# backtato/ai-video-detector

Hardware: AMD Instinct MI355X
Metric: sampled frames/sec analysed (1080p30 60 s clip, 2 fps sampling) (higher is better)
Workload: dtype u8 pixels; f32/f64 Farneback (cv2's own types); 1 GPU; BASELINE.json configs[1]: 1080p30 60 s clip, 2 fps sampling, one clip per GPU per step; frames_per_clip=120, height=1080, width=1920, clips_in_flight_per_gpu=3, fb_mode=fast+rerun, fb_wide160=2, parallelism=single GPU, rccl_ranks_seen=1

## Files before the change

ai-video-detector_amd/csrc/avd_capi.hip:

```cpp
#include <algorithm>
#include <cstdlib>
#include <atomic>
#include <cstring>
#include <new>
#include <thread>
#include "avd_internal.h"

namespace {

constexpr int kFbChunk = 128;
constexpr int kFbChunkMax = 512;

struct TableBlob {
    std::vector<uint8_t> bytes;
    template <typename T>
    size_t push(const std::vector<T>& v)
    {
        size_t off = (bytes.size() + 15) / 16 * 16;
        bytes.resize(off + v.size() * sizeof(T));
        std::memcpy(bytes.data() + off, v.data(), v.size() * sizeof(T));
        return off;
    }
};

// ... 741 lines not shown
        avd_ctx* c;
        ~Uncount() { if (c->counted_in_flight) { c->counted_in_flight = 0; g_calls_in_flight.fetch_sub(1, std::memory_order_relaxed); } }
    } uncount{ctx};
    HIP_TRY(ctx, hipSetDevice(ctx->device));
    if (ctx->tail.active) {
        const hipError_t e = ctx->tail_registered ? wait_helping(ctx, ctx->tail_ev) : hipStreamSynchronize(ctx->stream);
        tail_unregister(ctx);
        if (e != hipSuccess) { ctx->tail.active = 0; ctx->pending_out = nullptr; ctx->pending_n = 0; ctx->err = hipGetErrorString(e); return AVD_ERR_DEVICE; }
        if (ctx->tail.active) ctx->tail_rc = tail_settle(ctx);
    }
    if (ctx->tail_rc) {
        const int rc = ctx->tail_rc;
        ctx->tail_rc = 0; ctx->pending_out = nullptr; ctx->pending_n = 0;
        return rc;
    }
    HIP_TRY(ctx, wait_helping(ctx, nullptr));
    if (ctx->pending_out) {
        const avd_frame_record* const got = ctx->ws.h_rec + ctx->pending_off;
        std::memcpy(ctx->pending_out, got, sizeof(avd_frame_record) * ctx->pending_n);
        ctx->last_rerun = 0;
        for (int i = 0; i < ctx->pending_n; i++) ctx->last_rerun += got[i].reserved != 0;
        ctx->pending_out = nullptr; ctx->pending_n = 0;
    }
    if (ctx->profiling && ctx->kmark_used > 1 && ctx->kmark_id[ctx->kmark_used - 1] == AVD_K_COUNT) {
        for (float& v : ctx->kernel_ms) v = 0.f;
        for (int i = 0; i + 1 < ctx->kmark_used; i++) {
            float ms = 0.f;
            if (ctx->kmark_id[i] < AVD_K_COUNT && hipEventElapsedTime(&ms, ctx->kmark_at[i], ctx->kmark_at[i + 1]) == hipSuccess)
                ctx->kernel_ms[ctx->kmark_id[i]] += ms;
        }
        ctx->kmark_incomplete = ctx->kmark_overflow;
    }
    kmark_reset(ctx);
    if (ctx->profiling && ctx->stage_marks == 5) {
        for (int i = 0; i < 4; i++) {
            float ms = 0.f;
            if (hipEventElapsedTime(&ms, ctx->stage_ev[i], ctx->stage_ev[i + 1]) == hipSuccess) ctx->stage_ms[i] = ms;
        }
        float sum[2] = {0.f, 0.f}; int cnt[2] = {0, 0};
        for (int i = 0; i + 1 < ctx->kern_ev_used; i += 2) {
            float ms = 0.f;
            if (hipEventElapsedTime(&ms, ctx->kern_ev[i], ctx->kern_ev[i + 1]) == hipSuccess) { sum[(i >> 1) & 1] += ms; cnt[(i >> 1) & 1]++; }
        }
        for (int k = 0; k < 2; k++) ctx->stage_ms[4 + k] = cnt[k] ? sum[k] / cnt[k] : 0.f;
        ctx->stage_marks = 0;
    }
    return AVD_OK;
}

static int impl_timer_start(avd_ctx* ctx)
{
    if (!ctx) return AVD_ERR_ARG;
    HIP_TRY(ctx, hipEventRecord(ctx->ev0, ctx->stream));
    return AVD_OK;
}

static int impl_timer_stop(avd_ctx* ctx, float* elapsed_ms)
{
    if (!ctx || !elapsed_ms) return AVD_ERR_ARG;
    HIP_TRY(ctx, hipEventRecord(ctx->ev1, ctx->stream));
    HIP_TRY(ctx, hipEventSynchronize(ctx->ev1));
    HIP_TRY(ctx, hipEventElapsedTime(elapsed_ms, ctx->ev0, ctx->ev1));
    return AVD_OK;
}

static int impl_set_profiling(avd_ctx* ctx, int enable)
{
    if (!ctx) return AVD_ERR_ARG;
    ctx->profiling = enable != 0;
    return AVD_OK;
}

static int impl_stage_ms(avd_ctx* ctx, int stage, float* ms)
{
    if (!ctx || !ms || stage < 0 || stage > 5) return AVD_ERR_ARG;
    *ms = ctx->stage_ms[stage];
    return AVD_OK;
}

static int impl_kernel_ms(avd_ctx* ctx, int id, float* ms)
{
    if (!ctx || !ms || id < 0 || id >= AVD_K_COUNT) return AVD_ERR_ARG;
    if (ctx->kmark_incomplete) { ctx->err = "avd_kernel_ms: the profiled call had more kernel regions than the library records (96): split it"; return AVD_ERR_ARG; }
    *ms = ctx->kernel_ms[id];
    return AVD_OK;
}

static int64_t impl_debug_fetch(avd_ctx* ctx, const char* name, void* out, size_t out_bytes)
{
    if (!ctx || !name || !out) return AVD_ERR_ARG;
    Workspace& ws = ctx->ws;
    const int n = ctx->last_n;
    const void* src = nullptr;
    size_t bytes = 0;
    auto level = [&](const char* prefix) -> int {
        const size_t L = std::strlen(prefix);
        if (std::strncmp(name, prefix, L) == 0 && name[L] >= '0' && name[L] < '0' + AVD_FB_LEVELS && name[L + 1] == 0)
            return name[L] - '0';
        return -1;
    };
    int k;
    {
        const IngestRecord& in = ctx->ingest;
        const char* const no_launch = "no ingest kernel was launched on this context";
        const char* const no_call = "no ingest call has run on this context";
        const struct { const char* name; const void* p; size_t bytes; bool recorded; const char* missing; const char* type; } host_state[] = {
            {"ingest_plan", &in.plan, sizeof in.plan, in.launched != 0, no_launch, nullptr},
            {"ingest_rotate", &in.rotate, sizeof in.rotate, in.launched != 0, no_launch, "int32[1]"},
            {"ingest_range", &in.range, sizeof in.range, in.launched != 0, no_launch, "int32[1]"},
            {"ingest_format", &in.format, sizeof in.format, in.launched != 0, no_launch, "int32[1]"},
            {"ingest_list", in.list, sizeof in.list, in.launched != 0, no_launch, "int32[2]"},
            {"stage_copies", &in.stage_copies, sizeof in.stage_copies, in.stage_copies >= 0, no_call, "int64[1]"},
            {"stage_bytes", &in.stage_bytes, sizeof in.stage_bytes, in.stage_bytes >= 0, no_call, "int64[1]"},
        };
        for (const auto& e : host_state) {
            if (std::strcmp(name, e.name) != 0) continue;
            if (!e.recorded) { ctx->err = std::string(e.name) + " not recorded yet: " + e.missing; return AVD_ERR_ARG; }
            if (e.type && out_bytes < e.bytes) { ctx->err = std::string(e.name) + " is " + e.type; return AVD_ERR_ARG; }
            bytes = std::min(e.bytes, out_bytes);
            std::memcpy(out, e.p, bytes);
            return (int64_t)bytes;
        }
    }
    if (std::strcmp(name, "cnn_plan") == 0) {
        if (!ctx->cnn_plan_valid) { ctx->err = "cnn_plan not recorded yet: no CNN forward has run on this context"; return AVD_ERR_ARG; }
        bytes = std::min(sizeof(ctx->cnn_plan), out_bytes);
        std::memcpy(out, ctx->cnn_plan, bytes);
        return (int64_t)bytes;
    }
    if (std::strcmp(name, "cnn_tap") == 0) {
        HIP_TRY(ctx, hipSetDevice(ctx->device));
        return cnn_tap_fetch(ctx, out, out_bytes);
    }
    if (std::strncmp(name, "audio_", 6) == 0) {
        const bool plan = std::strcmp(name + 6, "plan") == 0, xw = std::strcmp(name + 6, "xw") == 0, mag = std::strcmp(name + 6, "mag") == 0;
        if (!plan && !xw && !mag) { ctx->err = "unknown debug buffer"; return AVD_ERR_ARG; }
        if (!ctx->audio_plan_valid) { ctx->err = "audio_plan / audio_xw / audio_mag not recorded yet: no avd_audio_features call has run on this context"; return AVD_ERR_ARG; }
        if (plan) {
            if (out_bytes < sizeof(ctx->audio_plan)) { ctx->err = "audio_plan is int32[4]"; return AVD_ERR_ARG; }
            std::memcpy(out, ctx->audio_plan, sizeof(ctx->audio_plan));
            return (int64_t)sizeof(ctx->audio_plan);
        }
        const size_t nwin = (size_t)ctx->audio_plan[0], win = (size_t)ctx->audio_plan[1];
        if (!ws.d_audio_buf) { ctx->err = "buffer not allocated yet"; return AVD_ERR_ARG; }
        src = xw ? ws.d_audio_buf.p : ws.d_audio_buf.p + nwin * win;
        bytes = (xw ? nwin * win : nwin * (win / 2 + 1)) * sizeof(double);
    }
    else if (std::strcmp(name, "area") == 0) { src = ws.d_area; bytes = (size_t)n * 1024; }
    else if (std::strcmp(name, "small") == 0) { src = ws.d_small; bytes = (size_t)n * AVD_NPIX; }
    else if ((k = level("pyr")) >= 0 && k == 0 && ctx->fb_fold_blur) { ctx->err = "pyr0 does not exist while fb_fold_blur is on (the polynomial expansion forms the 320-px blur itself)"; return AVD_ERR_ARG; }
    else if ((k = level("pyr")) >= 0) { src = ws.d_pyr[k]; bytes = (size_t)std::min(n, ws.fb_cap + 1) * (AVD_NPIX >> (2 * k)) * 4; }
    else if ((k = level("poly")) >= 0) { src = ws.d_poly[k]; bytes = (size_t)std::min(n, ws.fb_cap + 1) * 5 * (AVD_NPIX >> (2 * k)) * 4; }
    else if ((k = level("flow")) >= 0) { src = ws.fb_holds.flow[k] ? ws.fb_holds.flow[k] : ws.d_flow[k]; bytes = (size_t)std::min(std::max(n - 1, 0), ws.fb_cap) * 2 * (AVD_NPIX >> (2 * k)) * 4; }
    else if (std::strcmp(name, "vs0") == 0) { src = ws.d_vs0; bytes = fb_two_scratch_size((size_t)ws.fb_cap).vs0 * sizeof(double); }
    else { ctx->err = "unknown debug buffer"; return AVD_ERR_ARG; }
    if (!src) { ctx->err = "buffer not allocated yet"; return AVD_ERR_ARG; }
    bytes = std::min(bytes, out_bytes);
    HIP_TRY(ctx, hipSetDevice(ctx->device));
    HIP_TRY(ctx, hipStreamSynchronize(ctx->stream));
    HIP_TRY(ctx, hipMemcpy(out, src, bytes, hipMemcpyDeviceToHost));
    return (int64_t)bytes;
}

static int impl_wait_stream(avd_ctx* ctx, void* producer)
{
    if (!ctx) return AVD_ERR_ARG;
    HIP_TRY(ctx, hipSetDevice(ctx->device));
    HIP_TRY(ctx, hipEventRecord(ctx->ev_in, (hipStream_t)producer));
    HIP_TRY(ctx, hipStreamWaitEvent(ctx->stream, ctx->ev_in, 0));
    return AVD_OK;
}

static int impl_release_workspace(avd_ctx* ctx)
{
    if (!ctx) return AVD_ERR_ARG;
    HIP_TRY(ctx, hipSetDevice(ctx->device));
    if (int e = impl_synchronize(ctx)) return e;
    ctx->ws = Workspace{};
    ctx->rec_n = 0;
    return AVD_OK;
}

static int impl_set_option(avd_ctx* ctx, const char* name, int value)
{
    if (!ctx || !name) return AVD_ERR_ARG;
    const Option* o = find_option(ctx, name, true);
    if (!o) return AVD_ERR_ARG;
    if (!o->norm(value)) { ctx->err = o->refused; return AVD_ERR_ARG; }
    if (o->act) o->act(ctx, value);
    else ctx->*o->field = value;
    return AVD_OK;
}

static int impl_get_option(avd_ctx* ctx, const char* name, int* value)
{
    if (!ctx || !name || !value) return AVD_ERR_ARG;
    const Option* o = find_option(ctx, name, false);
    if (!o) return AVD_ERR_ARG;
    *value = o->read ? o->read(ctx) : ctx->*o->field;
    return AVD_OK;
}

template <typename F>
static int time_reps(avd_ctx* ctx, int reps, F&& launch, float* out_ms)
{
    HIP_TRY(ctx, hipEventRecord(ctx->ev0, ctx->stream));
    for (int r = 0; r < reps; r++)
        if (int e = launch()) return e;
    HIP_TRY(ctx, hipEventRecord(ctx->ev1, ctx->stream));
    HIP_TRY(ctx, hipEventSynchronize(ctx->ev1));
    float ms = 0.f;
    HIP_TRY(ctx, hipEventElapsedTime(&ms, ctx->ev0, ctx->ev1));
    *out_ms = ms / reps;
    return 0;
}

static int impl_cnn_set_weights(avd_ctx* ctx, const uint16_t* w, size_t n_w, const float* b, size_t n_b)
{
    if (!ctx || !w || !b) return AVD_ERR_ARG;
    size_t want_w = 0, want_b = 0;
    cnn_param_counts(&want_w, &want_b);
    if (n_w != want_w || n_b != want_b) { ctx->err = "avd_cnn_set_weights: parameter counts differ from avd_cnn_param_counts"; return AVD_ERR_ARG; }
    HIP_TRY(ctx, hipSetDevice(ctx->device));
    return cnn_set_weights(ctx, w, b);
}

static int impl_cnn_forward(avd_ctx* ctx, const uint8_t* bgr, int mem, int n, int h, int w, int64_t row_stride, int64_t frame_stride,
                            float* logits, int reps, float* forward_ms)
{
    if (!ctx) return AVD_ERR_ARG;
    if ((!bgr || !logits) && n > 0) { ctx->err = "null pointer"; return AVD_ERR_ARG; }
    if (n < 0 || h < 2 || w < 2 || row_stride < (int64_t)w * 3) { ctx->err = "bad frame geometry"; return AVD_ERR_ARG; }
    if (n == 0) return AVD_OK;
    HIP_TRY(ctx, hipSetDevice(ctx->device));
    Workspace& ws = ctx->ws;
    if (!ctx->weights.d_cnn_w) { ctx->err = "avd_cnn_set_weights has not been called"; return AVD_ERR_ARG; }
    const int kChunk = ctx->cnn_chunk;
    if (ctx->cnn_tap && (n > kChunk || reps > 0)) { ctx->err = "avd_cnn_forward: with option cnn_tap set, one pass (n <= cnn_chunk) and no timing repetitions"; return AVD_ERR_ARG; }
    if (int e = cnn_reserve(ctx, std::min(n, kChunk))) return e;
    const uint8_t* d_bgr = nullptr;
    if (int e = stage_input(ctx, bgr, mem, plane_span(frame_stride, n, row_stride, h, (size_t)w * 3), &d_bgr)) return e;
    float total_ms = 0.f;
    for (int f0 = 0; f0 < n; f0 += kChunk) {
        const int m = std::min(kChunk, n - f0);
        const uint8_t* src = d_bgr + (size_t)frame_stride * f0;
        auto forward = [&] { return launch_cnn_forward(ctx, src, m, h, w, row_stride, frame_stride); };
        if (int e = forward()) return e;
        if (reps > 0 && forward_ms) {
            float ms = 0.f;
            if (int e = time_reps(ctx, reps, forward, &ms)) return e;
            total_ms += ms;
        }
        HIP_TRY(ctx, hipMemcpyAsync(logits + (size_t)f0 * 1000, ws.d_cnn_logits, sizeof(float) * (size_t)m * 1000, hipMemcpyDeviceToHost, ctx->stream));
    }
    if (reps > 0 && forward_ms) *forward_ms = total_ms;
    HIP_TRY(ctx, hipStreamSynchronize(ctx->stream));
    return AVD_OK;
}

static int impl_vit_set_weights(avd_ctx* ctx, const uint16_t* w_bf16, const float* bias)
{
    if (!ctx || !w_bf16) return AVD_ERR_ARG;
    HIP_TRY(ctx, hipSetDevice(ctx->device));
    Weights& wt = ctx->weights;
    if (int e = wt.d_vit_w.reserve(ctx, (size_t)768 * 768)) return e;
    if (int e = wt.d_vit_bias.reserve(ctx, (size_t)768)) return e;
    std::vector<uint16_t> blocked((size_t)768 * 768);
    gemm_block_operand(w_bf16, blocked.data(), 768, 768);
    HIP_TRY(ctx, hipMemcpyAsync(wt.d_vit_w, blocked.data(), sizeof(uint16_t) * 768 * 768, hipMemcpyHostToDevice, ctx->stream));
    if (bias) HIP_TRY(ctx, hipMemcpyAsync(wt.d_vit_bias, bias, sizeof(float) * 768, hipMemcpyHostToDevice, ctx->stream));
    wt.vit_has_bias = bias != nullptr;
    HIP_TRY(ctx, hipStreamSynchronize(ctx->stream));
    return AVD_OK;
}

static int impl_vit_patch_embed(avd_ctx* ctx, const uint8_t* bgr, int mem, int n, int h, int w, int64_t row_stride,
                                int64_t frame_stride, void* tokens, int tokens_mem, int tokens_bf16, int reps, float* gemm_ms)
{
    if (!ctx) return AVD_ERR_ARG;
    if ((!bgr || !tokens) && n > 0) { ctx->err = "null pointer"; return AVD_ERR_ARG; }
    if (n < 0 || h < 2 || w < 2 || row_stride < (int64_t)w * 3) { ctx->err = "bad frame geometry"; return AVD_ERR_ARG; }
    if (tokens_mem != AVD_MEM_HOST && tokens_mem != AVD_MEM_DEVICE) { ctx->err = "tokens_mem must be AVD_MEM_HOST or AVD_MEM_DEVICE"; return AVD_ERR_ARG; }
    if (n == 0) return AVD_OK;
    HIP_TRY(ctx, hipSetDevice(ctx->device));
    Workspace& ws = ctx->ws;
    const Weights& wt = ctx->weights;
    if (!wt.d_vit_w) { ctx->err = "avd_vit_set_weights has not been called"; return AVD_ERR_ARG; }
    const size_t m = (size_t)n * 196;
    const size_t m_pad = (m + kGemmRowPad - 1) / kGemmRowPad * kGemmRowPad;
    if (ws.d_vit_patches.cap < m_pad * 768) {
        if (int e = ws.d_vit_patches.reserve(ctx, m_pad * 768)) return e;
        auto zero_fill = [&]() -> int { HIP_TRY(ctx, hipMemsetAsync(ws.d_vit_patches, 0, m_pad * 768 * sizeof(uint16_t), ctx->stream)); return 0; };
        if (int e = zero_fill()) { ws.d_vit_patches.reset(); return e; }
    }
    void* d_tok = tokens;
    const size_t esz = tokens_bf16 ? sizeof(uint16_t) : sizeof(float);
    if (tokens_mem == AVD_MEM_HOST) {
        if (int e = ws.d_vit_tokens.reserve(ctx, m * 768)) return e;
        d_tok = ws.d_vit_tokens;
    }
    const uint8_t* d_bgr = nullptr;
    if (int e = stage_input(ctx, bgr, mem, plane_span(frame_stride, n, row_stride, h, (size_t)w * 3), &d_bgr)) return e;
    const float* d_bias = wt.vit_has_bias ? wt.d_vit_bias : nullptr;
    if (int e = launch_vit_patch_embed(ctx, d_bgr, n, h, w, row_stride, frame_stride, wt.d_vit_w, d_bias, d_tok, tokens_bf16, ws.d_vit_patches)) return e;
    if (reps > 0 && gemm_ms) {
        auto gemm = [&] { return launch_gemm_bf16_nt(ctx, ws.d_vit_patches, wt.d_vit_w, d_bias, d_tok, tokens_bf16, (int)m, 768, 768); };
// ... 345 lines not shown
```

ai-video-detector_amd/csrc/avd_farneback.hip:

```cpp
#include "avd_internal.h"
#include "avd_fb_device.h"

#pragma clang fp contract(off)

namespace {

constexpr int S = AVD_SMALL;

template <int K>
struct PyrGeo {
    static constexpr int WL = S >> K;
    static constexpr int NC = K == 0 ? S : 2 * WL;
    static constexpr int OFF = K == 0 ? 0 : (1 << K) / 2 - 1;
    static constexpr int TR = K >= 2 ? 4 : 8;
    static constexpr int TILES = WL / TR;
    static constexpr int KS = K == 3 ? 19 : (K == 2 ? 9 : 3), HALF = KS / 2;
    static constexpr int SROWS = K == 0 ? TR + 2 * HALF : ((TR - 1) << K) + 2 + 2 * HALF;
    static constexpr int PADX = 12, PS = S + 2 * PADX;
    static constexpr int SRC_BYTES = SROWS * PS, LDS_BYTES = SRC_BYTES + SROWS * NC * 4;
};
constexpr int cmax(int a, int b) { return a > b ? a : b; }
constexpr int cgcd(int a, int b) { return b == 0 ? a : cgcd(b, a % b); }

template <int PR>
struct PyrWalk {
    static constexpr int PER = PR / cgcd(256, PR), SG = 256 / cgcd(256, PR);
    __device__ static __forceinline__ void first(int tid, int& r, int& c)
    {
        r = 0; c = tid;
#pragma unroll
        for (int q = 1; q * PR < 256; q++)
            if (tid >= q * PR) { r = q; c = tid - q * PR; }
    }
    __device__ static __forceinline__ void next(int& r, int& c)
    {
        r += 256 / PR; c += 256 % PR;
        if (c >= PR) { c -= PR; r++; }
    }
};
constexpr int kPyrLds = cmax(cmax(PyrGeo<3>::LDS_BYTES, PyrGeo<2>::LDS_BYTES), cmax(PyrGeo<1>::LDS_BYTES, PyrGeo<0>::LDS_BYTES));

template <int K>
__device__ __forceinline__ void pyramid_body(char* lds, int blk, const uint8_t* __restrict__ small, const FbConsts* __restrict__ C,
                                             float* __restrict__ I, int n = 0, int* __restrict__ pairdiff = nullptr)
{
    using G = PyrGeo<K>;
    constexpr int WL = G::WL, NC = G::NC, OFF = G::OFF, TR = G::TR, KS = G::KS, HALF = G::HALF, SROWS = G::SROWS;
    constexpr int PADX = G::PADX, PS = G::PS;
    uint8_t (*src)[PS] = reinterpret_cast<uint8_t (*)[PS]>(lds);
    float (*rowf)[NC] = reinterpret_cast<float (*)[NC]>(lds + G::SRC_BYTES);
    const int tiles = WL / TR;
    const int f = blk / tiles, t = blk - f * tiles;
    const int tid = threadIdx.x;
    const int dy0 = t * TR;
    const int y_first = (K == 0 ? dy0 : (dy0 << K) + OFF) - HALF;
    const uint8_t* img = small + (int64_t)f * AVD_NPIX;
    const bool cmp = K == 1 && pairdiff != nullptr && f + 1 < n;
    int differs = 0;
    for (int it = tid; it < SROWS * (S / 4); it += 256) {
        const int r = it / (S / 4), c4 = it - r * (S / 4);
        const int y = reflect101(y_first + r, S);
        const unsigned v = reinterpret_cast<const unsigned*>(img + y * S)[c4];
        reinterpret_cast<unsigned*>(src[r] + PADX)[c4] = v;
        if (K == 1 && cmp) differs |= v != reinterpret_cast<const unsigned*>(img + AVD_NPIX + y * S)[c4];
    }
    for (int it = tid; it < SROWS * 2 * HALF; it += 256) {
        const int r = it / (2 * HALF), i = it - r * (2 * HALF);
        const uint8_t* g = img + reflect101(y_first + r, S) * S;
        if (i < HALF) src[r][PADX - 1 - i] = g[1 + i];
        else src[r][PADX + S + (i - HALF)] = g[S - 2 - (i - HALF)];
    }
    if (K == 1 && cmp) {
        const int any = __syncthreads_or(differs);
        if (tid == 0) pairdiff[f * tiles + t] = any;
    } else
        __syncthreads();
    float kw[KS];
#pragma unroll
    for (int q = 0; q < KS; q++) kw[q] = C->gk[K][q];
    if (KS == 3) {
        static_assert(KS != 3 || NC == S, "the 3-tap scales filter whole rows");
        using W = PyrWalk<S / 4>;
        typedef float f4 __attribute__((ext_vector_type(4)));
        const unsigned* wp0[W::PER]; f4* dst0[W::PER]; int r0[W::PER];
        {
            int r, c4;
            W::first(tid, r, c4);
#pragma unroll
            for (int i = 0; i < W::PER; i++) {
                r0[i] = r;
                wp0[i] = reinterpret_cast<const unsigned*>(src[r] + PADX + 4 * c4);
                dst0[i] = reinterpret_cast<f4*>(&rowf[r][4 * c4]);
                W::next(r, c4);
            }
        }
        for (int sb = 0; sb < SROWS; sb += W::SG) {
#pragma unroll
            for (int i = 0; i < W::PER; i++) {
                if (256 * i >= SROWS * (S / 4) || r0[i] + sb >= SROWS) continue;
                const unsigned* wp = wp0[i] + sb * (PS / 4);
                const unsigned pw = wp[-1], cwd = wp[0], nw = wp[1];
                const float b[6] = {(float)(pw >> 24), (float)(cwd & 0xFFu), (float)((cwd >> 8) & 0xFFu), (float)((cwd >> 16) & 0xFFu),
                                    (float)(cwd >> 24), (float)(nw & 0xFFu)};
                f4 o;
#pragma unroll
                for (int e = 0; e < 4; e++) o[e] = __builtin_fmaf(b[e + 1], kw[1], (b[e] + b[e + 2]) * kw[0]);
                dst0[i][sb * (NC / 4)] = o;
            }
        }
    } else {
        using W = PyrWalk<NC>;
        constexpr int NW = (KS + 3) / 4;
        const unsigned* wp0[W::PER]; float* dst0[W::PER]; int r0[W::PER], sh0[W::PER];
        {
            int r, j;
            W::first(tid, r, j);
#pragma unroll
            for (int i = 0; i < W::PER; i++) {
                const int x = K == 0 ? j : ((j >> 1) << K) + OFF + (j & 1);
                const int base = PADX + x - HALF;
                r0[i] = r; sh0[i] = base & 3;
                wp0[i] = reinterpret_cast<const unsigned*>(src[r] + (base & ~3));
                dst0[i] = &rowf[r][j];
                W::next(r, j);
            }
        }
        for (int sb = 0; sb < SROWS; sb += W::SG) {
#pragma unroll
            for (int i = 0; i < W::PER; i++) {
                if (256 * i >= SROWS * NC || r0[i] + sb >= SROWS) continue;
                const unsigned* wp = wp0[i] + sb * (PS / 4);
                unsigned d[NW + 1];
#pragma unroll
                for (int q = 0; q <= NW; q++) d[q] = wp[q];
                float v = 0.f;
#pragma unroll
                for (int q = 0; q < NW; q++) {
                    const unsigned wv = __builtin_amdgcn_alignbyte(d[q + 1], d[q], sh0[i]);
#pragma unroll
                    for (int e = 0; e < 4; e++)
                        if (q * 4 + e < KS) v = __builtin_fmaf((float)((wv >> (8 * e)) & 0xFFu), kw[q * 4 + e], v);
                }
                dst0[i][sb * NC] = v;
            }
        }
    }
    __syncthreads();
    auto colf = [&](const float* c) {
        float sacc = __builtin_fmaf(c[0], kw[HALF], 0.f);
#pragma unroll
        for (int k = 1; k <= HALF; k++) sacc = __builtin_fmaf(c[k * NC] + c[-k * NC], kw[HALF + k], sacc);
        return sacc;
    };
    {
        using W = PyrWalk<WL>;
        float* out = I + ((int64_t)f * WL + dy0) * WL;
        int dyl, dx;
        W::first(tid, dyl, dx);
#pragma unroll
        for (int i = 0; i < W::PER; i++) {
            if (256 * i < TR * WL) {
                for (int y = dyl; y < TR; y += W::SG) {
                    float o;
                    if (K == 0) {
                        o = colf(&rowf[y + HALF][dx]);
                    } else {
                        const float* c = &rowf[(y << K) + HALF][2 * dx];
                        const float p00 = colf(c), p01 = colf(c + 1);
                        const float p10 = colf(c + NC), p11 = colf(c + NC + 1);
                        o = ((p00 + p01) + (p10 + p11)) * 0.25f;
                    }
                    out[y * WL + dx] = o;
                }
            }
            W::next(dyl, dx);
        }
    }
}

__global__ __launch_bounds__(256) void k_pyramid_all(const uint8_t* __restrict__ small, int n, const FbConsts* __restrict__ C,
                                                    float* __restrict__ I0, float* __restrict__ I1, float* __restrict__ I2,
                                                    float* __restrict__ I3, int* __restrict__ flags, int* __restrict__ pairdiff)
{
    static_assert(PyrGeo<1>::TILES == kPairDiffTiles, "avd_fbfast.hip reads one word per 160-px tile");
    __shared__ __align__(16) char lds[kPyrLds];
    if (flags && (int)(blockIdx.x * 256 + threadIdx.x) < n - 1) flags[blockIdx.x * 256 + threadIdx.x] = 0;
    const int n3 = n * PyrGeo<3>::TILES, n2 = n * PyrGeo<2>::TILES, n1 = n * PyrGeo<1>::TILES;
    int b = blockIdx.x;
    if (b < n3) { pyramid_body<3>(lds, b, small, C, I3); return; }
    b -= n3;
    if (b < n2) { pyramid_body<2>(lds, b, small, C, I2); return; }
    b -= n2;
    if (b < n1) { pyramid_body<1>(lds, b, small, C, I1, n, pairdiff); return; }
    if (I0) pyramid_body<0>(lds, b - n1, small, C, I0);
}

struct PolyPtrs { const float* I[AVD_FB_LEVELS]; float* R[AVD_FB_LEVELS]; const uint8_t* small; };

constexpr int kPolyRows = 16;
constexpr int kPolyQuads = 4 * (S / 4 + 10);
static_assert(AVD_FB_LEVELS == 4, "three walking scales and the one-row form of the coarsest");
__host__ __device__ constexpr int poly_wgs(int k) { return k < AVD_FB_LEVELS - 1 ? (S >> k) / kPolyRows : S >> (2 * k); }

typedef float pf4 __attribute__((ext_vector_type(4)));
typedef float pf2 __attribute__((ext_vector_type(2)));

__device__ __forceinline__ void polyexp_put(pf4* __restrict__ rowq, int x, int w, float t0, float t1, float t2)
{
    const pf4 t = {t0, t1, t1, t2};
    rowq[x + 5] = t;
    if (x == 0)
        for (int q = 0; q < 5; q++) rowq[q] = t;
    if (x == w - 1)
        for (int q = 0; q < 5; q++) rowq[w + 5 + q] = t;
}

__device__ __forceinline__ void polyexp_hpass(const pf4* __restrict__ rq, const float (&g)[6], const float (&xg)[6], const double (&gd)[6],
                                              const double (&xxgd)[6], double ig11, double ig03, double ig33, double ig55, float* __restrict__ o)
{
    const pf4 c = rq[0];
    double b1 = (double)(c.x * g[0]), b2 = 0, b3 = (double)(c.y * g[0]), b4 = 0, b5 = (double)(c.w * g[0]), b6 = 0;
#pragma unroll
    for (int q = 1; q <= 5; q++) {
        const pf4 p = rq[q], m = rq[-q];
        const pf2 s01 = p.xy + m.xy, d01 = p.xy - m.xy, s12 = p.zw + m.zw;
        const pf2 dx = d01 * pf2{xg[q], xg[q]};
        const pf2 sg = s12 * pf2{g[q], g[q]};
        const double tg = (double)s01.x;
        b1 = __builtin_fma(tg, gd[q], b1);
        b4 = __builtin_fma(tg, xxgd[q], b4);
        b2 += (double)dx.x;
        b3 += (double)sg.x;
        b6 += (double)dx.y;
        b5 += (double)sg.y;
    }
    o[0] = (float)(b3 * ig11);
    o[1] = (float)(b2 * ig11);
    o[2] = (float)(b1 * ig03 + b5 * ig33);
    o[3] = (float)(b1 * ig03 + b4 * ig33);
    o[4] = (float)(b6 * ig55);
}

template <int K, bool FOLD>
__device__ __forceinline__ void polyexp_rows(const float* __restrict__ img, const uint8_t* __restrict__ small, float* __restrict__ out, int y0,
                                             const FbConsts* __restrict__ C, pf4 (*rowb)[kPolyQuads], float (*outb)[S * 5])
{
    static_assert(!FOLD || K == 0, "only the 320-px scale forms its own blur");
    constexpr int w = S >> K, h = w, R = 1 << K, STEPS = kPolyRows / R;
    static_assert(R * (w + 10) <= kPolyQuads && h % kPolyRows == 0 && kPolyRows % R == 0, "a step's R rows fit one LDS buffer; whole bands");
    const int tid = threadIdx.x;
    const int sr = K == 0 ? 0 : tid / w, x = tid - sr * w;
    const int yb = y0 + sr;
    const int xs = x - 1 < 0 ? 0 : (x - 1 > w - 4 ? w - 4 : x - 1);
    const int shl = ((x == 0 ? 1 : x - 1) - xs) * 8, shc = (x - xs) * 8, shr = ((x == w - 1 ? w - 2 : x + 1) - xs) * 8;
    const float kx0 = C->gk[0][0], kx1 = C->gk[0][1], kx2 = C->gk[0][2];
    struct __attribute__((packed, aligned(1))) U4 { unsigned v; };
    auto hb = [&](int srow) __attribute__((always_inline)) {
        const int sr = srow < 0 ? -srow : (srow > h - 1 ? 2 * (h - 1) - srow : srow);
        const unsigned wd = reinterpret_cast<const U4*>(small + sr * w + xs)->v;
        const float l = (float)((wd >> shl) & 0xFFu), c = (float)((wd >> shc) & 0xFFu), r = (float)((wd >> shr) & 0xFFu);
        return __builtin_fmaf(c, kx1, (l + r) * kx0);
    };
    float hm = 0.f, h0 = 0.f, hp = 0.f;
    int rcur = -1000;
    auto blurred = [&](int r) __attribute__((always_inline)) {
        if (r != rcur) {
            if (r == rcur + 1) { hm = h0; h0 = hp; hp = hb(r + 1); }
            else { hm = hb(r - 1); h0 = hb(r); hp = hb(r + 1); }
            rcur = r;
        }
        return __builtin_fmaf(hp + hm, kx2, __builtin_fmaf(h0, kx1, 0.f));
    };
    auto pixel = [&](int r) __attribute__((always_inline)) { return FOLD ? blurred(r) : img[r * w + x]; };
    typedef float f4 __attribute__((ext_vector_type(4)));
    typedef float f2 __attribute__((ext_vector_type(2)));
    float g[6], xg[6], xxg[6];
    double gd[6], xxgd[6];
#pragma unroll
    for (int q = 0; q <= 5; q++) { g[q] = C->g[5 + q]; xg[q] = C->xg[5 + q]; xxg[q] = C->xxg[5 + q]; gd[q] = C->gd[q]; xxgd[q] = C->xxgd[q]; }
    const double ig11 = C->ig11, ig03 = C->ig03, ig33 = C->ig33, ig55 = C->ig55;
    float win[11 + kPolyRows - R];
#pragma unroll
    for (int q = 0; q < 10; q++) win[q] = pixel(min(max(yb - 5 + q, 0), h - 1));
    pf4* rowq[2] = {rowb[0] + sr * (w + 10), rowb[1] + sr * (w + 10)};
#pragma unroll
    for (int i = 0; i < STEPS; i++) {
        const int par = i & 1, o = R * i;
#pragma unroll
        for (int j = o + 11 - R; j <= o + 10; j++)
            if (j >= 10) win[j] = pixel(min(yb - 5 + j, h - 1));
        {
            f2 t02 = f2{win[o + 5] * g[0], 0.f};
            float t1 = 0.f;
#pragma unroll
            for (int q = 1; q <= 5; q++) {
                const float a = win[o + 5 - q], bb = win[o + 5 + q];
                const float p = a + bb;
                t02 = t02 + f2{g[q], xxg[q]} * f2{p, p};
                t1 = t1 + xg[q] * (bb - a);
            }
            polyexp_put(rowq[par], x, w, t02.x, t1, t02.y);
        }
        __syncthreads();
        if (i > 0) {
            f4* dst = reinterpret_cast<f4*>(out + (int64_t)(y0 + o - R) * w * 5);
            const f4* srcv = reinterpret_cast<const f4*>(outb[par ^ 1]);
            __builtin_nontemporal_store(srcv[tid], dst + tid);
            if (tid < S * 5 / 4 - 320) __builtin_nontemporal_store(srcv[tid + 320], dst + tid + 320);
        }
        polyexp_hpass(rowq[par] + x + 5, g, xg, gd, xxgd, ig11, ig03, ig33, ig55, outb[par] + tid * 5);
    }
    __syncthreads();
    {
        f4* dst = reinterpret_cast<f4*>(out + (int64_t)(y0 + kPolyRows - R) * w * 5);
        const f4* srcv = reinterpret_cast<const f4*>(outb[(STEPS - 1) & 1]);
        __builtin_nontemporal_store(srcv[tid], dst + tid);
        if (tid < S * 5 / 4 - 320) __builtin_nontemporal_store(srcv[tid + 320], dst + tid + 320);
    }
}

__global__ __launch_bounds__(320) void k_polyexp_all(PolyPtrs P, int n, const FbConsts* __restrict__ C)
{
    __shared__ pf4 rowb[2][kPolyQuads];
    __shared__ __align__(16) float outbb[2][S * 5];
    pf4* row = rowb[0];
    static_assert(8 * (S / 8 + 10) <= 2 * kPolyQuads, "the eight sub-rows of the coarsest scale fit");
    float* outb = outbb[0];
    int b = (int)blockIdx.x, k = 0, wgs = 0;
    for (; k < AVD_FB_LEVELS; k++) {
        wgs = n * poly_wgs(k);
        const int cnt = ((wgs + 7) >> 3) << 3;
// ... 336 lines not shown
```

Measured before the change: 145,100 frames/s.

## Reuse horizontally filtered halo rows across two vertical steps in pyramid levels 2-3

```diff
diff --git a/ai-video-detector_amd/csrc/avd_capi.hip b/ai-video-detector_amd/csrc/avd_capi.hip
--- a/ai-video-detector_amd/csrc/avd_capi.hip
+++ b/ai-video-detector_amd/csrc/avd_capi.hip
@@ -917,6 +917,7 @@
     else if ((k = level("pyr")) >= 0) { src = ws.d_pyr[k]; bytes = (size_t)std::min(n, ws.fb_cap + 1) * (AVD_NPIX >> (2 * k)) * 4; }
     else if ((k = level("poly")) >= 0) { src = ws.d_poly[k]; bytes = (size_t)std::min(n, ws.fb_cap + 1) * 5 * (AVD_NPIX >> (2 * k)) * 4; }
     else if ((k = level("flow")) >= 0) { src = ws.fb_holds.flow[k] ? ws.fb_holds.flow[k] : ws.d_flow[k]; bytes = (size_t)std::min(std::max(n - 1, 0), ws.fb_cap) * 2 * (AVD_NPIX >> (2 * k)) * 4; }
+    else if (std::strcmp(name, "pairdiff") == 0) { src = ws.d_pairdiff; bytes = (size_t)std::min(std::max(n - 1, 0), ws.fb_cap) * kPairDiffTiles * sizeof(int); }
     else if (std::strcmp(name, "vs0") == 0) { src = ws.d_vs0; bytes = fb_two_scratch_size((size_t)ws.fb_cap).vs0 * sizeof(double); }
     else { ctx->err = "unknown debug buffer"; return AVD_ERR_ARG; }
     if (!src) { ctx->err = "buffer not allocated yet"; return AVD_ERR_ARG; }
diff --git a/ai-video-detector_amd/csrc/avd_farneback.hip b/ai-video-detector_amd/csrc/avd_farneback.hip
--- a/ai-video-detector_amd/csrc/avd_farneback.hip
+++ b/ai-video-detector_amd/csrc/avd_farneback.hip
@@ -13,11 +13,17 @@
     static constexpr int NC = K == 0 ? S : 2 * WL;
     static constexpr int OFF = K == 0 ? 0 : (1 << K) / 2 - 1;
     static constexpr int TR = K >= 2 ? 4 : 8;
-    static constexpr int TILES = WL / TR;
+    static constexpr int STEPS = K >= 2 ? 2 : 1, BAND = STEPS * TR;
+    static constexpr int TILES = WL / BAND;
     static constexpr int KS = K == 3 ? 19 : (K == 2 ? 9 : 3), HALF = KS / 2;
     static constexpr int SROWS = K == 0 ? TR + 2 * HALF : ((TR - 1) << K) + 2 + 2 * HALF;
+    static constexpr int NEW = K == 0 ? TR : TR << K, KEEP = SROWS - NEW;
     static constexpr int PADX = 12, PS = S + 2 * PADX;
     static constexpr int SRC_BYTES = SROWS * PS, LDS_BYTES = SRC_BYTES + SROWS * NC * 4;
+    static constexpr int FILTERED_PCT = TILES * (SROWS + (STEPS - 1) * NEW) * 100 / S;
+    static_assert(WL % BAND == 0 && (K == 0 || FILTERED_PCT <= 120), "whole bands; a source row is filtered at most 1.2 times per frame");
+    static_assert(STEPS == 1 || (KEEP * NC <= 4 * 256 && SRC_BYTES % 16 == 0 && (NEW * NC) % 4 == 0 && (KEEP * NC) % 4 == 0),
+                  "the rows a step takes over move as one 16-byte piece per lane");
 };
 constexpr int cmax(int a, int b) { return a > b ? a : b; }
 constexpr int cgcd(int a, int b) { return b == 0 ? a : cgcd(b, a % b); }
@@ -40,49 +46,71 @@
 };
 constexpr int kPyrLds = cmax(cmax(PyrGeo<3>::LDS_BYTES, PyrGeo<2>::LDS_BYTES), cmax(PyrGeo<1>::LDS_BYTES, PyrGeo<0>::LDS_BYTES));
 
+typedef float pyr_f4 __attribute__((ext_vector_type(4)));
+typedef float pyr_f2 __attribute__((ext_vector_type(2)));
+
 template <int K>
-__device__ __forceinline__ void pyramid_body(char* lds, int blk, const uint8_t* __restrict__ small, const FbConsts* __restrict__ C,
-                                             float* __restrict__ I, int n = 0, int* __restrict__ pairdiff = nullptr)
+__device__ __forceinline__ void pyramid_step(char* lds, const uint8_t* __restrict__ img, const float (&kw)[PyrGeo<K>::KS], float* __restrict__ out,
+                                             int y_first, int rb, pyr_f4& kept, bool more, int* __restrict__ diffword)
 {
     using G = PyrGeo<K>;
     constexpr int WL = G::WL, NC = G::NC, OFF = G::OFF, TR = G::TR, KS = G::KS, HALF = G::HALF, SROWS = G::SROWS;
     constexpr int PADX = G::PADX, PS = G::PS;
     uint8_t (*src)[PS] = reinterpret_cast<uint8_t (*)[PS]>(lds);
     float (*rowf)[NC] = reinterpret_cast<float (*)[NC]>(lds + G::SRC_BYTES);
-    const int tiles = WL / TR;
-    const int f = blk / tiles, t = blk - f * tiles;
     const int tid = threadIdx.x;
-    const int dy0 = t * TR;
-    const int y_first = (K == 0 ? dy0 : (dy0 << K) + OFF) - HALF;
-    const uint8_t* img = small + (int64_t)f * AVD_NPIX;
-    const bool cmp = K == 1 && pairdiff != nullptr && f + 1 < n;
+    const bool cmp = K == 1 && diffword != nullptr;
+    static_assert(K != 1 || G::STEPS == 1, "the pair-identity word is formed by a tile that loads all its source rows in one step");
+    static_assert(HALF + 1 < S, "a source row is reflected at most once");
+    auto row_at = [&](int r) -> unsigned { const int y = y_first + r; return (unsigned)(y < 0 ? -y : (y >= S ? 2 * S - 2 - y : y)) * S; };
+    constexpr int NLD = (SROWS * (S / 4) + 255) / 256, NBD = (SROWS * 2 * HALF + 255) / 256;
+    const int nld = (SROWS - rb) * (S / 4), nbd = (SROWS - rb) * 2 * HALF;
+    constexpr int NBATCH = 8;
     int differs = 0;
-    for (int it = tid; it < SROWS * (S / 4); it += 256) {
-        const int r = it / (S / 4), c4 = it - r * (S / 4);
-        const int y = reflect101(y_first + r, S);
-        const unsigned v = reinterpret_cast<const unsigned*>(img + y * S)[c4];
-        reinterpret_cast<unsigned*>(src[r] + PADX)[c4] = v;
-        if (K == 1 && cmp) differs |= v != reinterpret_cast<const unsigned*>(img + AVD_NPIX + y * S)[c4];
-    }
-    for (int it = tid; it < SROWS * 2 * HALF; it += 256) {
-        const int r = it / (2 * HALF), i = it - r * (2 * HALF);
-        const uint8_t* g = img + reflect101(y_first + r, S) * S;
-        if (i < HALF) src[r][PADX - 1 - i] = g[1 + i];
-        else src[r][PADX + S + (i - HALF)] = g[S - 2 - (i - HALF)];
+#pragma unroll
+    for (int e0 = 0; e0 < NLD; e0 += NBATCH) {
+        const bool last = e0 + NBATCH >= NLD;
+        unsigned v[NBATCH], vn[K == 1 ? NBATCH : 1];
+        uint8_t bv[NBD];
+#pragma unroll
+        for (int e = e0; e < NLD && e < e0 + NBATCH; e++) {
+            const int it = tid + 256 * e, q = it / (S / 4), c4 = it - q * (S / 4);
+            if (it >= nld) continue;
+            const unsigned at = row_at(rb + q) + 4u * c4;
+            v[e - e0] = *reinterpret_cast<const unsigned*>(img + at);
+            if (K == 1 && cmp) vn[e - e0] = *reinterpret_cast<const unsigned*>(img + (at + AVD_NPIX));
+        }
+#pragma unroll
+        for (int e = 0; e < NBD; e++) {
+            const int it = tid + 256 * e, q = it / (2 * HALF), i = it - q * (2 * HALF);
+            if (!last || it >= nbd) continue;
+            bv[e] = img[row_at(rb + q) + (unsigned)(i < HALF ? 1 + i : S - 2 - (i - HALF))];
+        }
+#pragma unroll
+        for (int e = e0; e < NLD && e < e0 + NBATCH; e++) {
+            const int it = tid + 256 * e, q = it / (S / 4), c4 = it - q * (S / 4);
+            if (it >= nld) continue;
+            reinterpret_cast<unsigned*>(src[rb + q] + PADX)[c4] = v[e - e0];
+            if (K == 1 && cmp) differs |= v[e - e0] != vn[e - e0];
+        }
+#pragma unroll
+        for (int e = 0; e < NBD; e++) {
+            const int it = tid + 256 * e, q = it / (2 * HALF), i = it - q * (2 * HALF);
+            if (!last || it >= nbd) continue;
+            src[rb + q][i < HALF ? PADX - 1 - i : PADX + S + (i - HALF)] = bv[e];
+        }
+        __builtin_amdgcn_sched_barrier(0);
     }
     if (K == 1 && cmp) {
         const int any = __syncthreads_or(differs);
-        if (tid == 0) pairdiff[f * tiles + t] = any;
+        if (tid == 0) *diffword = any;
     } else
         __syncthreads();
-    float kw[KS];
-#pragma unroll
-    for (int q = 0; q < KS; q++) kw[q] = C->gk[K][q];
+    if (G::STEPS > 1 && rb && tid < G::KEEP * NC / 4) reinterpret_cast<pyr_f4*>(&rowf[0][0])[tid] = kept;
     if (KS == 3) {
         static_assert(KS != 3 || NC == S, "the 3-tap scales filter whole rows");
         using W = PyrWalk<S / 4>;
-        typedef float f4 __attribute__((ext_vector_type(4)));
-        const unsigned* wp0[W::PER]; f4* dst0[W::PER]; int r0[W::PER];
+        const unsigned* wp0[W::PER]; pyr_f4* dst0[W::PER]; int r0[W::PER];
         {
             int r, c4;
             W::first(tid, r, c4);
@@ -90,11 +118,11 @@
             for (int i = 0; i < W::PER; i++) {
                 r0[i] = r;
                 wp0[i] = reinterpret_cast<const unsigned*>(src[r] + PADX + 4 * c4);
-                dst0[i] = reinterpret_cast<f4*>(&rowf[r][4 * c4]);
+                dst0[i] = reinterpret_cast<pyr_f4*>(&rowf[r][4 * c4]);
                 W::next(r, c4);
             }
         }
-        for (int sb = 0; sb < SROWS; sb += W::SG) {
+        for (int sb = rb; sb < SROWS; sb += W::SG) {
 #pragma unroll
             for (int i = 0; i < W::PER; i++) {
                 if (256 * i >= SROWS * (S / 4) || r0[i] + sb >= SROWS) continue;
@@ -102,46 +130,46 @@
                 const unsigned pw = wp[-1], cwd = wp[0], nw = wp[1];
                 const float b[6] = {(float)(pw >> 24), (float)(cwd & 0xFFu), (float)((cwd >> 8) & 0xFFu), (float)((cwd >> 16) & 0xFFu),
                                     (float)(cwd >> 24), (float)(nw & 0xFFu)};
-                f4 o;
+                pyr_f4 o;
 #pragma unroll
                 for (int e = 0; e < 4; e++) o[e] = __builtin_fmaf(b[e + 1], kw[1], (b[e] + b[e + 2]) * kw[0]);
                 dst0[i][sb * (NC / 4)] = o;
             }
         }
     } else {
-        using W = PyrWalk<NC>;
-        constexpr int NW = (KS + 3) / 4;
-        const unsigned* wp0[W::PER]; float* dst0[W::PER]; int r0[W::PER], sh0[W::PER];
+        static_assert(KS == 3 || (K >= 2 && NC == 2 * WL), "the long filters run at the decimated scales, where the columns are pairs");
+        using W = PyrWalk<WL>;
+        constexpr int B0 = PADX + OFF - HALF, SH = B0 & 3, NW = (SH + KS + 1 + 3) / 4;
+        const unsigned* wp0[W::PER]; pyr_f2* dst0[W::PER]; int r0[W::PER];
         {
-            int r, j;
-            W::first(tid, r, j);
+            int r, jp;
+            W::first(tid, r, jp);
 #pragma unroll
             for (int i = 0; i < W::PER; i++) {
-                const int x = K == 0 ? j : ((j >> 1) << K) + OFF + (j & 1);
-                const int base = PADX + x - HALF;
-                r0[i] = r; sh0[i] = base & 3;
-                wp0[i] = reinterpret_cast<const unsigned*>(src[r] + (base & ~3));
-                dst0[i] = &rowf[r][j];
-                W::next(r, j);
+                r0[i] = r;
+                wp0[i] = reinterpret_cast<const unsigned*>(src[r] + (B0 & ~3) + (jp << K));
+                dst0[i] = reinterpret_cast<pyr_f2*>(&rowf[r][2 * jp]);
+                W::next(r, jp);
             }
         }
-        for (int sb = 0; sb < SROWS; sb += W::SG) {
+        for (int sb = rb; sb < SROWS; sb += W::SG) {
 #pragma unroll
             for (int i = 0; i < W::PER; i++) {
-                if (256 * i >= SROWS * NC || r0[i] + sb >= SROWS) continue;
+                if (256 * i >= SROWS * WL || r0[i] + sb >= SROWS) continue;
                 const unsigned* wp = wp0[i] + sb * (PS / 4);
-                unsigned d[NW + 1];
-#pragma unroll
-                for (int q = 0; q <= NW; q++) d[q] = wp[q];
-                float v = 0.f;
-#pragma unroll
-                for (int q = 0; q < NW; q++) {
-                    const unsigned wv = __builtin_amdgcn_alignbyte(d[q + 1], d[q], sh0[i]);
-#pragma unroll
-                    for (int e = 0; e < 4; e++)
-                        if (q * 4 + e < KS) v = __builtin_fmaf((float)((wv >> (8 * e)) & 0xFFu), kw[q * 4 + e], v);
+                unsigned d[NW];
+#pragma unroll
+                for (int q = 0; q < NW; q++) d[q] = wp[q];
+                float b[KS + 1];
+#pragma unroll
+                for (int q = 0; q <= KS; q++) b[q] = (float)((d[(SH + q) >> 2] >> (8 * ((SH + q) & 3))) & 0xFFu);
+                float v0 = 0.f, v1 = 0.f;
+#pragma unroll
+                for (int q = 0; q < KS; q++) {
+                    v0 = __builtin_fmaf(b[q], kw[q], v0);
+                    v1 = __builtin_fmaf(b[q + 1], kw[q], v1);
                 }
-                dst0[i][sb * NC] = v;
+                dst0[i][sb * (NC / 2)] = pyr_f2{v0, v1};
             }
         }
     }
@@ -154,7 +182,6 @@
     };
     {
         using W = PyrWalk<WL>;
-        float* out = I + ((int64_t)f * WL + dy0) * WL;
         int dyl, dx;
         W::first(tid, dyl, dx);
 #pragma unroll
@@ -165,10 +192,24 @@
                     if (K == 0) {
                         o = colf(&rowf[y + HALF][dx]);
                     } else {
-                        const float* c = &rowf[(y << K) + HALF][2 * dx];
-                        const float p00 = colf(c), p01 = colf(c + 1);
-                        const float p10 = colf(c + NC), p11 = colf(c + NC + 1);
-                        o = ((p00 + p01) + (p10 + p11)) * 0.25f;
+                        const pyr_f2* c = reinterpret_cast<const pyr_f2*>(&rowf[y << K][2 * dx]);
+                        float w[2][2 * HALF + 2];
+#pragma unroll
+                        for (int q = 0; q < 2 * HALF + 2; q++) {
+                            const pyr_f2 v = c[q * (NC / 2)];
+                            w[0][q] = v.x; w[1][q] = v.y;
+                        }
+                        float p[2][2];
+#pragma unroll
+                        for (int a = 0; a < 2; a++)
+#pragma unroll
+                            for (int e = 0; e < 2; e++) {
+                                float sacc = __builtin_fmaf(w[e][HALF + a], kw[HALF], 0.f);
+#pragma unroll
+                                for (int k = 1; k <= HALF; k++) sacc = __builtin_fmaf(w[e][HALF + a + k] + w[e][HALF + a - k], kw[HALF + k], sacc);
+                                p[a][e] = sacc;
+                            }
+                        o = ((p[0][0] + p[0][1]) + (p[1][0] + p[1][1])) * 0.25f;
                     }
                     out[y * WL + dx] = o;
                 }
@@ -176,7 +217,29 @@
             W::next(dyl, dx);
         }
     }
-}
+    if (G::STEPS > 1 && more && tid < G::KEEP * NC / 4) kept = reinterpret_cast<const pyr_f4*>(&rowf[G::NEW][0])[tid];
+}
+
+template <int K>
+__device__ __forceinline__ void pyramid_body(char* lds, int blk, const uint8_t* __restrict__ small, const FbConsts* __restrict__ C,
+                                             float* __restrict__ I, int n = 0, int* __restrict__ pairdiff = nullptr)
+{
+    using G = PyrGeo<K>;
+    constexpr int WL = G::WL;
+    const int f = blk / G::TILES, t = blk - f * G::TILES;
+    const int dy0 = t * G::BAND;
+    const uint8_t* img = small + (int64_t)f * AVD_NPIX;
+    float* out = I + ((int64_t)f * WL + dy0) * WL;
+    int* diffword = K == 1 && pairdiff != nullptr && f + 1 < n ? pairdiff + blk : nullptr;
+    float kw[G::KS];
+#pragma unroll
+    for (int q = 0; q < G::KS; q++) kw[q] = C->gk[K][q];
+    const int y_first = (K == 0 ? dy0 : (dy0 << K) + G::OFF) - G::HALF;
+    pyr_f4 kept = {0.f, 0.f, 0.f, 0.f};
+    for (int step = 0; step < G::STEPS; step++)
+        pyramid_step<K>(lds, img, kw, out + step * G::TR * WL, y_first + step * G::NEW, step ? G::KEEP : 0, kept, step + 1 < G::STEPS, diffword);
+}
+
 
 __global__ __launch_bounds__(256) void k_pyramid_all(const uint8_t* __restrict__ small, int n, const FbConsts* __restrict__ C,
                                                     float* __restrict__ I0, float* __restrict__ I1, float* __restrict__ I2,
```

Measured after the change: 147,100 frames/s, median of 6. 1.4% higher.
